# li-kunyi/dns-slam

Measured on AMD Instinct MI355X. Metric: ray-samples/s, higher is better.
Workload: dtype f32 (MLP products as 3 x f16 split-operand MFMA / 6 x bf16 for weight gradients, f32 accumulate: error <= fp32 fma chain)

## Files before the change

### dns_slam_amd/csrc/mlp_split.hip

```cpp
#include <cstdlib>
#include "mlp_split.hpp"

namespace dns {
namespace sp {
#ifdef DNS_BWD_TRACE
unsigned long long* g_bwd_trace = nullptr;
#endif

template <int NN, int NL, int PREC, bool XS = false>
__global__ __launch_bounds__(256, 2) void mlp_fwd_kernel(FwdArgs a) {
  extern __shared__ __attribute__((aligned(16))) unsigned char lds[];
  mlp_fwd_body<NN, NL, PREC, XS>(a, blockIdx.x, lds);
}

struct DwinArgs {
  const float* dh1;
  const float* x;
  uint32_t ldx;
  XSeg seg;
  uint32_t n_in, n_in_w;
  float* d_params;
  uint32_t n_slots;
  const int32_t* row_index;
  const int32_t* tile_group;
  uint32_t param_stride, tiles_per_block;
};

template <int NN, int IT, int PREC>
__global__ __launch_bounds__(256, 2) void mlp_dwin_kernel(DwinArgs a) {
  constexpr int NT = NN / 32;
  extern __shared__ __attribute__((aligned(16))) unsigned char lds[];
  float* stg_base = reinterpret_cast<float*>(lds);
  const uint32_t lane = threadIdx.x & 63u, wave = threadIdx.x >> 6;
  int* rows_lds = reinterpret_cast<int*>(stg_base + wave * STG_WAVE_FLOATS + STG_FLOATS);
  const uint32_t n_in = a.n_in;
  const uint32_t n_btiles = (a.n_slots + 127u) / 128u;
  const uint32_t bt0 = blockIdx.x * a.tiles_per_block;
  const uint32_t bt1 = min(bt0 + a.tiles_per_block, n_btiles);
  auto group_of = [&](uint32_t t) -> int { return a.tile_group ? a.tile_group[t] : 0; };
  const uint32_t ch = lane & 31u, pt8 = 8u * (lane >> 5);
  f32x16 acc[NT][IT];
  for (uint32_t run0 = bt0; run0 < bt1;) {
    const int grp = group_of(run0);
    uint32_t run1 = run0 + 1;
    while (run1 < bt1 && group_of(run1) == grp) ++run1;
    if (grp < 0) {
      run0 = run1;
      continue;
    }
#pragma unroll
    for (int i = 0; i < NT; ++i)
#pragma unroll
      for (int j = 0; j < IT; ++j) acc[i][j] = zero16();
    for (uint32_t bt = run0; bt < run1; ++bt) {
      const uint32_t slot0 = bt * 128u + wave * 32u;
      tile_rows_publish(rows_lds, a.row_index, slot0, a.n_slots, lane);
      Frag3 fa[NT][2];
#pragma unroll
      for (int t = 0; t < NT; ++t)
#pragma unroll
        for (int s = 0; s < 2; ++s) {
          float v[8];
#pragma unroll
          for (int j = 0; j < 8; ++j) {
            const uint32_t slot = slot0 + 16u * s + pt8 + j;
            v[j] = a.dh1[(size_t)min(slot, a.n_slots - 1u) * NN + 32 * t + ch];
          }
#pragma unroll
          for (int j = 0; j < 8; ++j) v[j] = (slot0 + 16u * s + pt8 + j) < a.n_slots ? v[j] : 0.f;
          fa[t][s] = split8_bf3(v);
        }
#pragma unroll
      for (int ct = 0; ct < IT; ++ct) {
        const uint32_t col_raw = 32u * ct + ch;
        const bool col_ok = col_raw < n_in;
        const uint32_t col = col_ok ? col_raw : n_in - 1u;
        const bool second = a.seg.x2 != nullptr && col >= a.seg.n_in1;
        const float* base = second ? a.seg.x2 + (col - a.seg.n_in1) : a.x + col;
        const uint32_t ld = second ? a.seg.ldx2 : a.ldx;
#pragma unroll
        for (int s = 0; s < 2; ++s) {
          float v[8];
          int rowv[8];
#pragma unroll
          for (int j = 0; j < 8; ++j) rowv[j] = rows_lds[16 * s + pt8 + j];
#pragma unroll
          for (int j = 0; j < 8; ++j) v[j] = base[(size_t)max(rowv[j], 0) * ld];
#pragma unroll
          for (int j = 0; j < 8; ++j) v[j] = (rowv[j] >= 0 && col_ok) ? v[j] : 0.f;
          const Frag3 fb = split8_bf3(v);
#pragma unroll
          for (int t = 0; t < NT; ++t) acc[t][ct] = mma_pt<PREC>(fa[t][s], fb, acc[t][ct]);
        }
      }
    }
    __syncthreads();
    {
      float* dW = a.d_params + (size_t)grp * a.param_stride;
#pragma unroll 1
      for (uint32_t k = 0; k < (uint32_t)IT; ++k) {
        const uint32_t jj = (k + blockIdx.x) % (uint32_t)IT;
#pragma unroll
        for (int j = 0; j < IT; ++j) {
          if (jj == (uint32_t)j) {
#pragma unroll
            for (int i = 0; i < NT; ++i)
              flush_tile(acc[i][j], dW + (size_t)(32 * i) * a.n_in_w + 32 * j, a.n_in_w, 32u, n_in > 32u * j ? n_in - 32u * j : 0u, stg_base, wave, lane);
          }
        }
      }
    }
    run0 = run1;
  }
}

template <int NN, int NL>
static bool set_fwd_attrs() {
  return hipFuncSetAttribute((const void*)mlp_fwd_kernel<NN, NL, 3>, hipFuncAttributeMaxDynamicSharedMemorySize, MAX_DYN_LDS) == hipSuccess &&
         hipFuncSetAttribute((const void*)mlp_fwd_kernel<NN, NL, 1>, hipFuncAttributeMaxDynamicSharedMemorySize, MAX_DYN_LDS) == hipSuccess &&
         hipFuncSetAttribute((const void*)mlp_fwd_kernel<NN, NL, 3, true>, hipFuncAttributeMaxDynamicSharedMemorySize, MAX_DYN_LDS) == hipSuccess &&
         hipFuncSetAttribute((const void*)mlp_fwd_kernel<NN, NL, 1, true>, hipFuncAttributeMaxDynamicSharedMemorySize, MAX_DYN_LDS) == hipSuccess;
}

static int split_init_attrs() {
  const bool ok = set_fwd_attrs<32, 1>() && set_fwd_attrs<32, 2>() && set_fwd_attrs<64, 1>() && set_fwd_attrs<64, 2>();
  if (!ok) {
    set_error("dns_init: hipFuncSetAttribute failed for the split-operand MLP kernels");
    return DNS_E_LAUNCH;
  }
  return DNS_OK;
}
static AttrRegistrar split_attr_registrar(split_init_attrs);

}

int launch_mlp_fwd_split(const float* x, uint32_t ldx, const float* x2, uint32_t ldx2, uint32_t n_in1, const float* params,
                         uint32_t n_in, uint32_t n_out, uint32_t n_neurons, uint32_t n_hidden_layers, float* y, uint32_t ldy,
                         uint32_t n_slots, const int32_t* row_index, const int32_t* tile_group, uint32_t param_stride,
                         float* h_save, bool fp16_single, const unsigned char* prep, uint32_t prep_stride, const sp::XsIn* xs,
                         hipStream_t st, uint32_t n_in_w) {
  using namespace sp;
  FwdArgs a;
  a.n_in_w = n_in_w ? n_in_w : n_in;
  a.xs = xs ? *xs : XsIn{};
  a.prep = prep; a.prep_stride = prep_stride;
  a.x = x; a.ldx = ldx; a.seg = {x2, ldx2, x2 ? n_in1 : n_in}; a.params = params; a.n_in = n_in; a.n_out = n_out;
  a.y = y; a.ldy = ldy; a.n_slots = n_slots; a.row_index = row_index; a.tile_group = tile_group; a.param_stride = param_stride;
  a.h_save = h_save;
  a.err = device_error_word();
  DNS_REQUIRE((row_index ? 0ull : (uint64_t)n_slots) * ldy * 4ull < (uint64_t)BUF_LIMIT &&
                  (!h_save || 2ull * n_slots * n_neurons * 4ull < (uint64_t)BUF_LIMIT),
              "dns_mlp_fwd: %u slots x %u output floats per row exceed the 2 GiB per matrix this kernel addresses", n_slots, ldy);
  const uint32_t n_btiles = (n_slots + 127u) / 128u;
  uint32_t tpb = (n_btiles + 511u) / 512u;
  if (tpb < 1) tpb = 1;
  a.tiles_per_block = tpb;
  const uint32_t blocks = (n_btiles + tpb - 1) / tpb;
#define LAUNCH_FWD(NN, NL)                                                                                           \
  {                                                                                                                  \
    const size_t lds_bytes = FwdLds<NN, NL>::total(n_in, n_out, 4);                                                  \
    if (xs) {                                                                                                        \
      if (fp16_single) DNS_LAUNCH((mlp_fwd_kernel<NN, NL, 1, true>), dim3(blocks), dim3(256), lds_bytes, st, a);     \
      else DNS_LAUNCH((mlp_fwd_kernel<NN, NL, 3, true>), dim3(blocks), dim3(256), lds_bytes, st, a);                 \
    } else if (fp16_single) DNS_LAUNCH((mlp_fwd_kernel<NN, NL, 1>), dim3(blocks), dim3(256), lds_bytes, st, a);      \
    else DNS_LAUNCH((mlp_fwd_kernel<NN, NL, 3>), dim3(blocks), dim3(256), lds_bytes, st, a);                         \
  }
  if (n_neurons == 32 && n_hidden_layers == 1) LAUNCH_FWD(32, 1)
  else if (n_neurons == 32 && n_hidden_layers == 2) LAUNCH_FWD(32, 2)
  else if (n_neurons == 64 && n_hidden_layers == 1) LAUNCH_FWD(64, 1)
  else LAUNCH_FWD(64, 2)
#undef LAUNCH_FWD
  return check_launch("dns_mlp_fwd");
}

int launch_mlp_bwd_split(const float* x, uint32_t ldx, const float* x2, uint32_t ldx2, uint32_t n_in1, const float* dy,
                         uint32_t lddy, const float* params, uint32_t n_in, uint32_t n_out, uint32_t n_neurons,
                         uint32_t n_hidden_layers, float* d_x, uint32_t lddx, float* d_x2, uint32_t lddx2, float* d_params,
                         float* ws, uint32_t n_slots, const int32_t* row_index, const int32_t* tile_group,
                         uint32_t param_stride, int acc1, int acc2, bool fp16_single, const unsigned char* prep, uint32_t prep_stride,
                         bool with_dwin, const float* h_saved, const sp::XsIn* xs, hipStream_t st, uint32_t n_in_w) {
  using namespace sp;
  BwdArgs a;
  a.n_in_w = n_in_w ? n_in_w : n_in;
  a.xs = xs ? *xs : XsIn{};
  a.h_saved = h_saved;
  a.prep = prep; a.prep_stride = prep_stride;
#ifdef DNS_BWD_TRACE
  a.trace = g_bwd_trace;
#endif
  a.x = x; a.ldx = ldx; a.seg = {x2, ldx2, x2 ? n_in1 : n_in}; a.dy = dy; a.lddy = lddy; a.params = params;
  a.n_in = n_in; a.n_out = n_out; a.dx = d_x; a.lddx = lddx;
  a.dseg = {(d_x && x2) ? d_x2 : nullptr, lddx2, (uint32_t)acc1 & 1u, (uint32_t)acc2, (uint32_t)acc1 >> 8};
  a.d_params = d_params; a.dh1 = d_params ? ws : nullptr;
  a.n_slots = n_slots; a.row_index = row_index; a.tile_group = tile_group; a.param_stride = param_stride;
  a.err = device_error_word();
  {
    uint64_t ld_max = lddy;
    if (d_x) ld_max = lddx > ld_max ? lddx : ld_max;
    if (d_x && x2 && d_x2) ld_max = lddx2 > ld_max ? lddx2 : ld_max;
    const uint64_t rows = row_index ? 0ull : (uint64_t)n_slots;
    DNS_REQUIRE(rows * ld_max * 4ull < (uint64_t)BUF_LIMIT && (uint64_t)n_slots * n_neurons * 4ull < (uint64_t)BUF_LIMIT &&
                    (uint64_t)n_slots * 4ull < (uint64_t)BUF_LIMIT,
                "dns_mlp_bwd: %u slots x %llu floats per row exceed the 2 GiB per matrix this kernel addresses", n_slots,
                (unsigned long long)ld_max);
  }
  const bool wide = !d_params && !tile_group && !h_saved;
  a.n_waves = wide ? 8u : 4u;
  const uint32_t bt_slots = 32u * a.n_waves;
  const uint32_t n_btiles = (n_slots + bt_slots - 1u) / bt_slots;
  uint32_t tpb = (n_btiles + 255u) / 256u;
  if (tpb < 1) tpb = 1;
  a.tiles_per_block = tpb;
  const uint32_t blocks = (n_btiles + tpb - 1) / tpb;
  int rc;
  if (n_neurons == 32 && n_hidden_layers == 1) rc = launch_bwd_32_1(a, blocks, fp16_single, st);
  else if (n_neurons == 32 && n_hidden_layers == 2) rc = launch_bwd_32_2(a, blocks, fp16_single, st);
  else if (n_neurons == 64 && n_hidden_layers == 1) rc = launch_bwd_64_1(a, blocks, fp16_single, st);
  else rc = launch_bwd_64_2(a, blocks, fp16_single, st);
  if (rc != DNS_OK || !d_params || !with_dwin) return rc;
  return launch_mlp_dwin(x, ldx, x2, ldx2, n_in1, n_in, n_neurons, n_hidden_layers, d_params, ws, n_slots, row_index, tile_group,
                         param_stride, fp16_single, st, n_in_w);
}

int launch_mlp_dwin(const float* x, uint32_t ldx, const float* x2, uint32_t ldx2, uint32_t n_in1, uint32_t n_in, uint32_t n_neurons,
                    uint32_t n_hidden_layers, float* d_params, const float* ws, uint32_t n_slots, const int32_t* row_index,
                    const int32_t* tile_group, uint32_t param_stride, bool fp16_single, hipStream_t st, uint32_t n_in_w) {
  using namespace sp;
  (void)n_hidden_layers;
  const uint32_t n_btiles = (n_slots + 127u) / 128u;
  DwinArgs d;
  d.dh1 = ws; d.x = x; d.ldx = ldx; d.seg = {x2, ldx2, x2 ? n_in1 : n_in}; d.n_in = n_in; d.n_in_w = n_in_w ? n_in_w : n_in; d.d_params = d_params; d.n_slots = n_slots;
  d.row_index = row_index; d.tile_group = tile_group; d.param_stride = param_stride;
  static const uint32_t dwin_blocks = [] { const char* e = getenv("DNS_DWIN_BLOCKS"); const long n = e ? atol(e) : 0; return (uint32_t)(n >= 64 && n <= 4096 ? n : 512); }();
  uint32_t tpb2 = (n_btiles + dwin_blocks - 1u) / dwin_blocks;
  if (tpb2 < 1) tpb2 = 1;
  d.tiles_per_block = tpb2;
  const uint32_t blocks2 = (n_btiles + tpb2 - 1) / tpb2;
  const size_t lds2 = 4 * STG_WAVE_FLOATS * sizeof(float);
  const uint32_t it = (n_in + 31u) / 32u;
#define LAUNCH_DWIN2(NN, IT)                                                                                          \
  {                                                                                                                   \
    if (fp16_single) DNS_LAUNCH((mlp_dwin_kernel<NN, IT, 1>), dim3(blocks2), dim3(256), lds2, st, d);        \
    else DNS_LAUNCH((mlp_dwin_kernel<NN, IT, 3>), dim3(blocks2), dim3(256), lds2, st, d);                     \
  }
#define LAUNCH_DWIN(NN)                  \
  {                                      \
    if (it <= 1) LAUNCH_DWIN2(NN, 1)     \
    else if (it == 2) LAUNCH_DWIN2(NN, 2) \
    else if (it == 3) LAUNCH_DWIN2(NN, 3) \
    else LAUNCH_DWIN2(NN, 4)             \
  }
  if (n_neurons == 32) LAUNCH_DWIN(32)
  else LAUNCH_DWIN(64)
#undef LAUNCH_DWIN
#undef LAUNCH_DWIN2
  return check_launch("dns_mlp_bwd(dW_in)");
}

static uint32_t prepared_fwd_bytes(uint32_t n_in, uint32_t n_out, uint32_t nn, uint32_t nl) {
  using namespace sp;
  uint32_t b;
  if (nn == 32 && nl == 1) b = FwdLds<32, 1>::misc(n_in, n_out);
  else if (nn == 32) b = FwdLds<32, 2>::misc(n_in, n_out);
  else if (nl == 1) b = FwdLds<64, 1>::misc(n_in, n_out);
  else b = FwdLds<64, 2>::misc(n_in, n_out);
  return b + 16u;
}
static uint32_t prepared_bwd_bytes(uint32_t n_in, uint32_t n_out, uint32_t nn, uint32_t nl) {
  using namespace sp;
  if (nn == 32 && nl == 1) return prepared_bwd_bytes_32_1(n_in, n_out);
  if (nn == 32) return prepared_bwd_bytes_32_2(n_in, n_out);
  if (nl == 1) return prepared_bwd_bytes_64_1(n_in, n_out);
  return prepared_bwd_bytes_64_2(n_in, n_out);
}
uint32_t mlp_prepared_fwd_bytes(uint32_t n_in, uint32_t n_out, uint32_t nn, uint32_t nl) { return prepared_fwd_bytes(n_in, n_out, nn, nl); }
uint32_t mlp_prepared_bytes(uint32_t n_in, uint32_t n_out, uint32_t nn, uint32_t nl) {
  return prepared_fwd_bytes(n_in, n_out, nn, nl) + prepared_bwd_bytes(n_in, n_out, nn, nl);
}
int launch_mlp_prepare(const float* params, uint32_t param_stride, uint32_t n_in, uint32_t n_out, uint32_t nn, uint32_t nl,
                       uint32_t n_sets, unsigned char* blob, hipStream_t st, uint32_t n_in_w) {
  using namespace sp;
  if (n_in_w == 0) n_in_w = n_in;
  const uint32_t stride = mlp_prepared_bytes(n_in, n_out, nn, nl), fb = prepared_fwd_bytes(n_in, n_out, nn, nl);
  if (nn == 32 && nl == 1) return prepare_32_1(params, param_stride, n_in, n_out, n_sets, blob, fb, stride, st, n_in_w);
  if (nn == 32) return prepare_32_2(params, param_stride, n_in, n_out, n_sets, blob, fb, stride, st, n_in_w);
  if (nl == 1) return prepare_64_1(params, param_stride, n_in, n_out, n_sets, blob, fb, stride, st, n_in_w);
  return prepare_64_2(params, param_stride, n_in, n_out, n_sets, blob, fb, stride, st, n_in_w);
}

}

#ifdef DNS_BWD_TRACE
extern "C" void dns_debug_bwd_trace(unsigned long long* buf) { dns::sp::g_bwd_trace = buf; }
#endif
```

Measured before the change: 172.9 million.

## Double-buffer dW_in operand tiles in LDS via async global-to-LDS DMA

Rewrites the input-weight gradient kernel to stage dh1 and gathered input rows into per-wave double-buffered LDS slots using global_load_lds, with explicit vmcnt waits so the next half-tile's loads overlap the current MFMA work. Row indices are also DMA'd ahead, and validity is tracked with a ballot mask. This targets the latency of scattered per-element global loads, at the cost of much larger LDS use, which lowers occupancy (one block per CU for NN=64/IT=4, fewer default blocks when LDS is large) and adds fragile manual waitcnt accounting.

```diff
diff --git a/dns_slam_amd/csrc/mlp_split.hip b/dns_slam_amd/csrc/mlp_split.hip
--- a/dns_slam_amd/csrc/mlp_split.hip
+++ b/dns_slam_amd/csrc/mlp_split.hip
@@ -1,3 +1,4 @@
+#include <algorithm>
 #include <cstdlib>
 #include "mlp_split.hpp"
 
@@ -12,6 +13,11 @@
   extern __shared__ __attribute__((aligned(16))) unsigned char lds[];
   mlp_fwd_body<NN, NL, PREC, XS>(a, blockIdx.x, lds);
 }
+
+constexpr uint32_t DWIN_XBLK = 1024u + 64u;
+constexpr uint32_t DWIN_ROWS_BYTES = 2u * 64u * 4u;
+__host__ __device__ constexpr uint32_t dwin_slot_bytes(uint32_t nn, uint32_t w16) { return 64u * nn + w16 * DWIN_XBLK; }
+__host__ __device__ constexpr uint32_t dwin_wave_bytes(uint32_t nn, uint32_t w16) { return 2u * dwin_slot_bytes(nn, w16) + DWIN_ROWS_BYTES; }
 
 struct DwinArgs {
   const float* dh1;
@@ -24,21 +30,73 @@
   const int32_t* row_index;
   const int32_t* tile_group;
   uint32_t param_stride, tiles_per_block;
+  uint32_t w16;
 };
 
+typedef __attribute__((address_space(3))) void* lds_ptr_t;
+template <uint32_t SIZE>
+__device__ __forceinline__ void lds_dma(const void* src, unsigned char* dst) {
+  static_assert(SIZE == 4 || SIZE == 16, "LDS-DMA widths used here: 4 and 16 bytes");
+  if constexpr (SIZE == 16) __builtin_amdgcn_global_load_lds(src, (lds_ptr_t)dst, 16, 0, 0);
+  else __builtin_amdgcn_global_load_lds(src, (lds_ptr_t)dst, 4, 0, 0);
+}
+__device__ __forceinline__ void wait_vm(uint32_t n) {
+  switch (n) {
+#define DNS_WVM(k) case k: asm volatile("s_waitcnt vmcnt(" #k ")" ::: "memory"); break;
+    DNS_WVM(1) DNS_WVM(2) DNS_WVM(3) DNS_WVM(4) DNS_WVM(5) DNS_WVM(6) DNS_WVM(7) DNS_WVM(8) DNS_WVM(9) DNS_WVM(10)
+    DNS_WVM(11) DNS_WVM(12) DNS_WVM(13) DNS_WVM(14)
+#undef DNS_WVM
+    default: asm volatile("s_waitcnt vmcnt(0)" ::: "memory"); break;
+  }
+}
+
 template <int NN, int IT, int PREC>
-__global__ __launch_bounds__(256, 2) void mlp_dwin_kernel(DwinArgs a) {
+__global__ __launch_bounds__(256, (NN == 64 && IT == 4) ? 1 : 2) void mlp_dwin_kernel(DwinArgs a) {
   constexpr int NT = NN / 32;
+  constexpr uint32_t DH_DMA = NN / 16;
+  constexpr uint32_t DH_BYTES = 64u * NN;
   extern __shared__ __attribute__((aligned(16))) unsigned char lds[];
   float* stg_base = reinterpret_cast<float*>(lds);
   const uint32_t lane = threadIdx.x & 63u, wave = threadIdx.x >> 6;
-  int* rows_lds = reinterpret_cast<int*>(stg_base + wave * STG_WAVE_FLOATS + STG_FLOATS);
-  const uint32_t n_in = a.n_in;
-  const uint32_t n_btiles = (a.n_slots + 127u) / 128u;
+  const uint32_t n_in = a.n_in, n_slots = a.n_slots, w16 = a.w16;
+  const uint32_t slot_bytes = dwin_slot_bytes(NN, w16);
+  unsigned char* area = lds + wave * dwin_wave_bytes(NN, w16);
+  unsigned char* rows_area = area + 2u * slot_bytes;
+  const uint32_t nd = DH_DMA + w16;
+  const bool table = a.row_index != nullptr;
+  const uint32_t n_btiles = (n_slots + 127u) / 128u;
   const uint32_t bt0 = blockIdx.x * a.tiles_per_block;
   const uint32_t bt1 = min(bt0 + a.tiles_per_block, n_btiles);
   auto group_of = [&](uint32_t t) -> int { return a.tile_group ? a.tile_group[t] : 0; };
   const uint32_t ch = lane & 31u, pt8 = 8u * (lane >> 5);
+  const uint32_t xr = lane >> 2, n_in4 = (n_in + 3u) & ~3u;
+
+  auto issue_rows = [&](uint32_t bt, uint32_t par) {
+    asm volatile("s_waitcnt lgkmcnt(0)" ::: "memory");
+    const uint32_t slot = min(bt * 128u + wave * 32u + ch, n_slots - 1u);
+    lds_dma<4>(a.row_index + slot, rows_area + par * 256u);
+  };
+  auto issue_half = [&](uint32_t bt, uint32_t s, unsigned char* buf, uint32_t par) {
+    asm volatile("s_waitcnt lgkmcnt(0)" ::: "memory");
+    const uint32_t sbase = bt * 128u + wave * 32u + 16u * s;
+#pragma unroll
+    for (uint32_t k = 0; k < DH_DMA; ++k) {
+      const uint32_t e = k * 256u + lane * 4u;
+      const uint32_t slot = min(sbase + e / NN, n_slots - 1u);
+      lds_dma<16>(a.dh1 + (size_t)slot * NN + e % NN, buf + k * 1024u);
+    }
+    const uint32_t slot = sbase + xr;
+    int row = (int)slot;
+    if (table) row = reinterpret_cast<const int*>(rows_area + par * 256u)[16u * s + xr];
+    row = (slot < n_slots && row >= 0) ? row : 0;
+    for (uint32_t b = 0; b < w16; ++b) {
+      const uint32_t col = min(16u * b + 4u * (lane & 3u), n_in4 - 4u);
+      const bool second = a.seg.x2 != nullptr && col >= a.seg.n_in1;
+      const float* src = second ? a.seg.x2 + (size_t)row * a.seg.ldx2 + (col - a.seg.n_in1) : a.x + (size_t)row * a.ldx + col;
+      lds_dma<16>(src, buf + DH_BYTES + b * DWIN_XBLK);
+    }
+  };
+
   f32x16 acc[NT][IT];
   for (uint32_t run0 = bt0; run0 < bt1;) {
     const int grp = group_of(run0);
@@ -52,46 +110,67 @@
     for (int i = 0; i < NT; ++i)
 #pragma unroll
       for (int j = 0; j < IT; ++j) acc[i][j] = zero16();
-    for (uint32_t bt = run0; bt < run1; ++bt) {
+    const uint32_t n_tiles = run1 - run0, n_half = 2u * n_tiles;
+    auto rows_exist = [&](uint32_t t) -> uint32_t { return (table && t < n_tiles) ? 1u : 0u; };
+    if (table) {
+      issue_rows(run0, 0u);
+      wait_vm(0u);
+    }
+    issue_half(run0, 0u, area, 0u);
+    if (rows_exist(1u)) issue_rows(run0 + 1u, 1u);
+    issue_half(run0, 1u, area + slot_bytes, 0u);
+    uint64_t xmask = 0;
+    for (uint32_t h = 0; h < n_half; ++h) {
+      const uint32_t t = h >> 1, s = h & 1u;
+      const uint32_t bt = run0 + t;
+      wait_vm(s == 0u ? rows_exist(t + 1u) + nd : (h + 1u < n_half ? nd : 0u));
       const uint32_t slot0 = bt * 128u + wave * 32u;
-      tile_rows_publish(rows_lds, a.row_index, slot0, a.n_slots, lane);
-      Frag3 fa[NT][2];
-#pragma unroll
-      for (int t = 0; t < NT; ++t)
-#pragma unroll
-        for (int s = 0; s < 2; ++s) {
-          float v[8];
-#pragma unroll
-          for (int j = 0; j < 8; ++j) {
-            const uint32_t slot = slot0 + 16u * s + pt8 + j;
-            v[j] = a.dh1[(size_t)min(slot, a.n_slots - 1u) * NN + 32 * t + ch];
-          }
-#pragma unroll
-          for (int j = 0; j < 8; ++j) v[j] = (slot0 + 16u * s + pt8 + j) < a.n_slots ? v[j] : 0.f;
-          fa[t][s] = split8_bf3(v);
+      if (s == 0u) {
+        int row = (int)(slot0 + ch);
+        if (table) row = reinterpret_cast<const int*>(rows_area + (t & 1u) * 256u)[ch];
+        xmask = __ballot(lane < 32u && slot0 + ch < n_slots && row >= 0);
+      }
+      unsigned char* buf = area + s * slot_bytes;
+      const uint32_t sb = slot0 + 16u * s;
+      const uint32_t m8 = (uint32_t)(xmask >> (16u * s + pt8)) & 0xffu;
+      float va[NT][8], vb[IT][8];
+#pragma unroll
+      for (int tt = 0; tt < NT; ++tt) {
+        const float* dh = reinterpret_cast<const float*>(buf) + pt8 * NN + 32 * tt + ch;
+#pragma unroll
+        for (int j = 0; j < 8; ++j) va[tt][j] = dh[j * NN];
+      }
+#pragma unroll
+      for (int ct = 0; ct < IT; ++ct) {
+        const uint32_t col = min(32u * ct + ch, n_in - 1u);
+        const float* xb = reinterpret_cast<const float*>(buf + DH_BYTES + (col >> 4) * DWIN_XBLK) + pt8 * 16u + (col & 15u);
+#pragma unroll
+        for (int j = 0; j < 8; ++j) vb[ct][j] = xb[16 * j];
+      }
+      if (h + 2u < n_half) {
+        if (s == 0u) {
+          if (table) wait_vm(nd);
+          issue_half(bt + 1u, 0u, buf, (t + 1u) & 1u);
+        } else {
+          if (rows_exist(t + 2u)) issue_rows(bt + 2u, t & 1u);
+          issue_half(bt + 1u, 1u, buf, (t + 1u) & 1u);
         }
+      }
+      Frag3 fa[NT];
+#pragma unroll
+      for (int tt = 0; tt < NT; ++tt) {
+#pragma unroll
+        for (int j = 0; j < 8; ++j) va[tt][j] = (sb + pt8 + j) < n_slots ? va[tt][j] : 0.f;
+        fa[tt] = split8_bf3(va[tt]);
+      }
 #pragma unroll
       for (int ct = 0; ct < IT; ++ct) {
-        const uint32_t col_raw = 32u * ct + ch;
-        const bool col_ok = col_raw < n_in;
-        const uint32_t col = col_ok ? col_raw : n_in - 1u;
-        const bool second = a.seg.x2 != nullptr && col >= a.seg.n_in1;
-        const float* base = second ? a.seg.x2 + (col - a.seg.n_in1) : a.x + col;
-        const uint32_t ld = second ? a.seg.ldx2 : a.ldx;
-#pragma unroll
-        for (int s = 0; s < 2; ++s) {
-          float v[8];
-          int rowv[8];
-#pragma unroll
-          for (int j = 0; j < 8; ++j) rowv[j] = rows_lds[16 * s + pt8 + j];
-#pragma unroll
-          for (int j = 0; j < 8; ++j) v[j] = base[(size_t)max(rowv[j], 0) * ld];
-#pragma unroll
-          for (int j = 0; j < 8; ++j) v[j] = (rowv[j] >= 0 && col_ok) ? v[j] : 0.f;
-          const Frag3 fb = split8_bf3(v);
-#pragma unroll
-          for (int t = 0; t < NT; ++t) acc[t][ct] = mma_pt<PREC>(fa[t][s], fb, acc[t][ct]);
-        }
+        const bool col_ok = 32u * ct + ch < n_in;
+#pragma unroll
+        for (int j = 0; j < 8; ++j) vb[ct][j] = (col_ok && ((m8 >> j) & 1u)) ? vb[ct][j] : 0.f;
+        const Frag3 fb = split8_bf3(vb[ct]);
+#pragma unroll
+        for (int tt = 0; tt < NT; ++tt) acc[tt][ct] = mma_pt<PREC>(fa[tt], fb, acc[tt][ct]);
       }
     }
     __syncthreads();
@@ -122,8 +201,19 @@
          hipFuncSetAttribute((const void*)mlp_fwd_kernel<NN, NL, 1, true>, hipFuncAttributeMaxDynamicSharedMemorySize, MAX_DYN_LDS) == hipSuccess;
 }
 
+template <int NN>
+static bool set_dwin_attrs() {
+  bool ok = true;
+  const void* k[8] = {(const void*)mlp_dwin_kernel<NN, 1, 3>, (const void*)mlp_dwin_kernel<NN, 2, 3>, (const void*)mlp_dwin_kernel<NN, 3, 3>,
+                      (const void*)mlp_dwin_kernel<NN, 4, 3>, (const void*)mlp_dwin_kernel<NN, 1, 1>, (const void*)mlp_dwin_kernel<NN, 2, 1>,
+                      (const void*)mlp_dwin_kernel<NN, 3, 1>, (const void*)mlp_dwin_kernel<NN, 4, 1>};
+  for (const void* f : k) ok = ok && hipFuncSetAttribute(f, hipFuncAttributeMaxDynamicSharedMemorySize, MAX_DYN_LDS) == hipSuccess;
+  return ok;
+}
+
 static int split_init_attrs() {
-  const bool ok = set_fwd_attrs<32, 1>() && set_fwd_attrs<32, 2>() && set_fwd_attrs<64, 1>() && set_fwd_attrs<64, 2>();
+  const bool ok = set_fwd_attrs<32, 1>() && set_fwd_attrs<32, 2>() && set_fwd_attrs<64, 1>() && set_fwd_attrs<64, 2>() &&
+                  set_dwin_attrs<32>() && set_dwin_attrs<64>();
   if (!ok) {
     set_error("dns_init: hipFuncSetAttribute failed for the split-operand MLP kernels");
     return DNS_E_LAUNCH;
@@ -231,12 +321,14 @@
   DwinArgs d;
   d.dh1 = ws; d.x = x; d.ldx = ldx; d.seg = {x2, ldx2, x2 ? n_in1 : n_in}; d.n_in = n_in; d.n_in_w = n_in_w ? n_in_w : n_in; d.d_params = d_params; d.n_slots = n_slots;
   d.row_index = row_index; d.tile_group = tile_group; d.param_stride = param_stride;
-  static const uint32_t dwin_blocks = [] { const char* e = getenv("DNS_DWIN_BLOCKS"); const long n = e ? atol(e) : 0; return (uint32_t)(n >= 64 && n <= 4096 ? n : 512); }();
+  d.w16 = (n_in + 15u) / 16u;
+  const size_t lds2 = std::max<size_t>(4u * dwin_wave_bytes(n_neurons, d.w16), 4 * STG_WAVE_FLOATS * sizeof(float));
+  static const long dwin_blocks_env = [] { const char* e = getenv("DNS_DWIN_BLOCKS"); const long n = e ? atol(e) : 0; return n >= 64 && n <= 4096 ? n : 0L; }();
+  const uint32_t dwin_blocks = dwin_blocks_env ? (uint32_t)dwin_blocks_env : (2u * lds2 <= (size_t)MAX_DYN_LDS ? 512u : 256u);
   uint32_t tpb2 = (n_btiles + dwin_blocks - 1u) / dwin_blocks;
   if (tpb2 < 1) tpb2 = 1;
   d.tiles_per_block = tpb2;
   const uint32_t blocks2 = (n_btiles + tpb2 - 1) / tpb2;
-  const size_t lds2 = 4 * STG_WAVE_FLOATS * sizeof(float);
   const uint32_t it = (n_in + 31u) / 32u;
 #define LAUNCH_DWIN2(NN, IT)                                                                                          \
   {                                                                                                                   \
```

After: 175.1 million, median of 6. 1.3% higher.
